# BaekMS/Sep-TFAnet-VAD

Hardware: AMD Instinct MI355X
Metric: utterances/sec/GPU (4s@8kHz, 2spk+VAD); SI-SDR within 0.01 dB of ref (higher is better)
Workload: dtype f16x3 (fp32-accurate); 1 GPU; cfg2 config_with_vad.json forward, B=64/GPU, N=32000 samples (4 s @ 8 kHz resampled to 16 kHz), T=126 frames; full forward: STFT, 24 TCN blocks, VAD, iSTFT, est (side attributes on read); global_batch=64, seq_len=32000, parallelism=dp1 (independent utterance shards, no data-path collective)

## Files before the change

sep-tfanet-vad_amd/csrc/api.hip:

```cpp
#include <hip/hip_runtime.h>
#include <hip/hip_fp16.h>

#include "build/build_id.h"

#include <algorithm>
#include <climits>
#include <cmath>
#include <cstdio>
#include <cstdlib>
#include <cstring>
#include <memory>
#include <mutex>
#include <numeric>
#include <string>
#include <unordered_map>
#include <vector>

#include <rocprofiler-sdk-roctx/roctx.h>

#include "../../include/sepvad.h"
#include "sepvad_internal.h"
#include "stoi_design.h"

using namespace sepvad;
// ... 48 lines not shown

Workspace ws_view(const Workspace& w, int b0, int Tp) {
  Workspace v = w;
  const size_t u = (size_t)b0 * Tp;
  v.X = w.X + u * NBIN; v.specdb = w.specdb + u * SPEC_LD; v.S0 = w.S0 + u * CH;
  v.O[0] = w.O[0] + u * CH; v.O[1] = w.O[1] + u * CH; v.A = w.A + u * CH; v.R = w.R + u * CH;
  v.masks = w.masks + u * MOUT_PAD;
  v.Dhi = w.Dhi + u * HID; v.Dlo = w.Dlo + u * HID; v.D32 = w.D32 + u * HID;
  v.colsum = w.colsum + u * (CH / TILE); v.rowsum = w.rowsum + (size_t)b0 * (Tp / TILE) * CH;
  v.at = w.at + u; v.af = w.af + (size_t)b0 * CH; v.vy = w.vy + u * 2 * 4; v.vad = w.vad + u * 2;
  v.vP = w.vP + u * 2 * HEAD_VAD_N;
  v.rec_gate = w.rec_gate + (size_t)b0 * (Tp / GATE_ROWS) * 2;
  v.rec_g1 = w.rec_g1 + (size_t)b0 * (Tp / TILE) * (CH / TILE) * 2;
  v.rec_dw = w.rec_dw + (size_t)b0 * (Tp / STAT_ROWS) * 2;
  v.rec_mom = w.rec_mom + (size_t)b0 * (Tp / STAT_ROWS) * NMOM;
  v.rec_hs = w.rec_hs + (size_t)b0 * (Tp / STAT_ROWS) * 2;
  v.rec_vad = w.rec_vad + (size_t)b0 * 2 * (Tp / VAD_ROWS) * 2;
  return v;
}

constexpr int MAX_SPLIT = 4;
constexpr int TCLK_RECS = 4096;

struct StreamCtx {
  void* stream = nullptr;
  Workspace ws;
  unsigned long long* tgran = nullptr;
  unsigned* terr = nullptr;
  unsigned* herr = nullptr;
  unsigned* herr_dev = nullptr;
  unsigned reported = 0;
  unsigned pending = 0;
  unsigned tsalt = 0;
  int last_B = 0, last_N = 0;
  long long seq = 0;
  unsigned long long used = 0;
};

}

struct sepvad_model {
  SepVadConfig cfg{};
  int device = 0;
  int nblk = 0;
  int prec = PREC_F16X3;
  float* dparams = nullptr;
  __half* dhalf = nullptr;
  std::vector<BlockOff> blk;
  size_t win_in = 0, win_out = 0, win_inv = 0, tw = 0;
  size_t ln_g = 0, ln_b = 0;
  PackedW wout;
  size_t out_g = 0, out_b = 0, bo = 0;
  PackedW wout_spk, vadw;
  size_t bo_spk = 0, out_nyw = 0, out_nyb = 0, vad_ny = 0;
  float vad_sx = 1.f;
  float out_a = 0.f;
  size_t v_w1 = 0, v_b1 = 0, v_g = 0, v_b = 0, v_w2 = 0;
  float v_a = 0.f, v_b2 = 0.f;
  size_t gate = 0;
  bool same_stft_window = true;
  int split = 1;
  hipStream_t sub[MAX_SPLIT] = {};
  hipEvent_t fork = nullptr, join[MAX_SPLIT] = {};
  bool fused = true;
  int tcn_cap = 0;
  int tcn_cap_p[4] = {};
  __half* twf = nullptr;
  __half* twq[3] = {};
  __half* twfq = nullptr;
  int lo8 = 2;
  int tcn_cap_q[3] = {};
  int tcn2_cap_p[4] = {};
  int tcn2_cap_q[3] = {};
  int gran_slots = 0;
  __half* twf16 = nullptr;
  __half* twbf = nullptr;
  float* twf32 = nullptr;
  float* tprm = nullptr;
  bool last_fused = false;
  float out_sx = 1.f;
  int last_nsl = 1;
  float* tdump = nullptr;
  std::vector<std::unique_ptr<StreamCtx>> ctx;
  std::mutex mu;
  unsigned long long use_clock = 0;
  long long fwd_seq = 0;
  int res_B = 0, res_N = 0;
  unsigned long long* kprobe = nullptr;
  unsigned long long* tprobe = nullptr;
  unsigned long long* tclk = nullptr;
  long long tclk_n = 0;
  bool timing = false;
  std::vector<hipEvent_t> ev;
  double gemm_ms = 0.0, g2_ms = 0.0, total_ms = 0.0;
  int gemm_launches = 0, g2_launches = 0;
  int probe_blk = -1;
  unsigned long long* probe = nullptr;
  size_t probe_n = 0;

  const float* P(size_t off) const { return dparams + off; }
  const __half* H(size_t off) const { return dhalf + off; }
};

namespace {

struct TensorMap {
  std::unordered_map<std::string, std::pair<const float*, int64_t>> m;
// ... 614 lines not shown
        const float* bb = get(q + convs[j] + ".bias", 1);
        BAIL();
        attp[4 * j + 0] = w[0]; attp[4 * j + 1] = w[1]; attp[4 * j + 2] = w[2]; attp[4 * j + 3] = bb[0];
      }
      const float* pt = get(q + ".prelu_t.weight", 1);
      const float* pf = get(q + ".prelu_f.weight", 1);
      BAIL();
      attp[16] = pt[0]; attp[17] = pf[0];
    }
    bo.attp = pk.add(attp);
    if (c.ln_mode == SEPVAD_LN_RECURSIVE) {
      const float* fa = get("TCN.ln_first_modules." + std::to_string(i) + ".weight", CH);
      const float* fb = get("TCN.ln_first_modules." + std::to_string(i) + ".bias", CH);
      const float* sa = get("TCN.ln_second_modules." + std::to_string(i) + ".weight", CH);
      const float* sb = get("TCN.ln_second_modules." + std::to_string(i) + ".bias", CH);
      BAIL();
      bo.lna_g = pk.add(fa, CH); bo.lna_b = pk.add(fb, CH);
      bo.lnb_g = pk.add(sa, CH); bo.lnb_b = pk.add(sb, CH);
      xbound = gn_bound(sa, sb, CH);
      for (int j = 0; j < 5; ++j) bo.wsum[j] = 0.0;
      for (int k = 0; k < CH; ++k) {
        const double g = fa[k], e = fb[k];
        bo.wsum[0] += g; bo.wsum[1] += e; bo.wsum[2] += e * e; bo.wsum[3] += g * e; bo.wsum[4] += g * g;
      }
    } else if (c.ln_mode == SEPVAD_LN_RESIDUAL) {
      const float* fa = get("TCN.ln_modules." + std::to_string(i) + ".weight", CH);
      const float* fb = get("TCN.ln_modules." + std::to_string(i) + ".bias", CH);
      BAIL();
      bo.lna_g = pk.add(fa, CH); bo.lna_b = pk.add(fb, CH);
      xbound += gn_bound(fa, fb, CH);
    } else {
      xbound = 0.0;
    }
    h->blk.push_back(bo);
  }
  {
    const float* oa = get("TCN.output.0.weight", 1);
    const float* og = get("TCN.output.1.weight", CH);
    const float* ob = get("TCN.output.1.bias", CH);
    const float* gg = get("TCN.output.2.weight_g", MOUT);
    const float* vv = get("TCN.output.2.weight_v", (int64_t)MOUT * CH);
    const float* bb = get("TCN.output.2.bias", MOUT);
    BAIL();
    h->out_a = oa[0];
    h->out_g = pk.add(og, CH);
    h->out_b = pk.add(ob, CH);
    const int eh = range_exp(gn_bound(og, ob, CH));
    h->out_sx = std::ldexp(1.f, -eh);
    const std::vector<float> wo = fold_wn(gg, vv, MOUT, CH);
    h->wout = pack_pointwise(pk, wo, MOUT, CH, MOUT_PAD, eh);
    std::vector<float> bpad(MOUT_PAD, 0.f);
    std::memcpy(bpad.data(), bb, MOUT * sizeof(float));
    h->bo = pk.add(bpad);
    std::vector<float> ws((size_t)MOUT_PAD * CH, 0.f), bs(MOUT_PAD, 0.f);
    for (int q = 0; q < 2; ++q)
      for (int i = 0; i < NBIN; ++i) {
        std::memcpy(&ws[((size_t)q * HEAD_SPK + i) * CH], &wo[((size_t)q * NBIN + i) * CH], CH * sizeof(float));
        bs[q * HEAD_SPK + i] = bb[q * NBIN + i];
      }
    h->wout_spk = pack_pointwise(pk, ws, MOUT_PAD, CH, MOUT_PAD, eh);
    h->bo_spk = pk.add(bs);
    std::vector<float> nyw((size_t)2 * CH), nyb(2);
    for (int q = 0; q < 2; ++q) {
      std::memcpy(&nyw[(size_t)q * CH], &wo[((size_t)q * NBIN + NBIN - 1) * CH], CH * sizeof(float));
      nyb[q] = bb[q * NBIN + NBIN - 1];
    }
    h->out_nyw = pk.add(nyw);
    h->out_nyb = pk.add(nyb);
  }
  if (c.final_vad) {
    const float* g1 = get("vad.common.conv1_1.weight_g", 4);
    const float* v1 = get("vad.common.conv1_1.weight_v", (int64_t)4 * NBIN * 5);
    const float* b1 = get("vad.common.conv1_1.bias", 4);
    const float* a = get("vad.common.relu_1.weight", 1);
    const float* gg = get("vad.common.BN_1.weight", 4);
    const float* gb = get("vad.common.BN_1.bias", 4);
    const float* g2 = get("vad.output_layer_vad.weight_g", 1);
    const float* v2 = get("vad.output_layer_vad.weight_v", 12);
    const float* b2 = get("vad.output_layer_vad.bias", 1);
    BAIL();
    const std::vector<float> w1 = fold_wn(g1, v1, 4, NBIN * 5);
    h->v_w1 = pk.add(w1);
    std::vector<float> wv((size_t)32 * HEAD_SPK, 0.f);
    for (int o = 0; o < 4; ++o)
      for (int c2 = 0; c2 < NBIN; ++c2)
        for (int k = 0; k < 5; ++k) wv[(size_t)(4 * k + o) * HEAD_SPK + c2] = w1[((size_t)o * NBIN + c2) * 5 + k];
    double mb = 0.0;
    {
      const std::vector<float> wo = fold_wn(get("TCN.output.2.weight_g", MOUT), get("TCN.output.2.weight_v", (int64_t)MOUT * CH), MOUT, CH);
      const float* ob2 = get("TCN.output.2.bias", MOUT);
      const double ab = gn_bound(get("TCN.output.1.weight", CH), get("TCN.output.1.bias", CH), CH);
      for (int r = 0; r < MOUT; ++r) {
        double sr = 0.0;
        for (int i = 0; i < CH; ++i) sr += std::fabs((double)wo[(size_t)r * CH + i]);
        mb = std::max(mb, sr * ab + std::fabs((double)ob2[r]));
      }
    }
    const int ev_ = range_exp(mb);
    h->vad_sx = std::ldexp(1.f, -ev_);
    h->vadw = pack_pointwise(pk, wv, HEAD_VAD_N, HEAD_SPK, 32, ev_);
    std::vector<float> vny(HEAD_VAD_N);
    for (int o = 0; o < 4; ++o)
      for (int k = 0; k < 5; ++k) vny[4 * k + o] = w1[((size_t)o * NBIN + NBIN - 1) * 5 + k];
    h->vad_ny = pk.add(vny);
    h->v_b1 = pk.add(b1, 4);
    h->v_a = a[0];
    h->v_g = pk.add(gg, 4);
    h->v_b = pk.add(gb, 4);
    h->v_w2 = pk.add(fold_wn(g2, v2, 1, 12));
    h->v_b2 = b2[0];
  }
  {
    std::vector<float> gw(12, 0.f);
    if (c.activity_input) {
      const float* w = get("activity_input.weight", 9);
      const float* bb = get("activity_input.bias", 1);
      const float* pa = get("prelu.weight", 1);
      BAIL();
      std::memcpy(gw.data(), w, 9 * sizeof(float));
      gw[9] = bb[0];
      gw[10] = pa[0];
// ... 201 lines not shown
    sa.window_db = h->same_stft_window ? sa.window : h->P(h->win_in);
    sa.X = w.X;
    sa.specdb = h->same_stft_window ? nullptr : w.specdb;
    sa.activity = c.activity_input; sa.gate_w = h->P(h->gate);
    sa.S0 = w.S0; sa.gate_rec = w.rec_gate;
    TailProbe tp(h, s, kn, "stft");
    sa.probe = tp.buf;
    HIPCHK(launch_stft_gate(sa, s));
    HIPCHK(tp.dump(B, Tp / (2 * GATE_ROWS)));
    if (out->spectrum) {
      GateArgs ga{};
      ga.B = B; ga.T = T; ga.Tp = Tp; ga.activity = c.activity_input;
      ga.X = h->same_stft_window ? w.X : nullptr; ga.specdb = w.specdb; ga.w = h->P(h->gate);
      ga.S0 = nullptr; ga.out_rec = nullptr;
      ga.spec_side = out->spectrum + (size_t)b0 * NBIN * T;
      HIPCHK(launch_gate(ga, s));
    }
  }
  stage.next("sepvad::tcn_head");
  const int G = (T + FR - 1) / FR;
  const bool use_fused = fused_ok(h, T);
  unsigned gsalt_lo = 0, gsalt_n = 0;
  h->last_fused = use_fused;
  const bool has_vad = c.final_vad && (!c.final_vad_masked_speakers || c.noisy_phase);
  const bool vad_in_head = use_fused && has_vad && !c.final_vad_masked_speakers;
  if (use_fused) {
    const int nsl = h->tdump ? 1 : tcn_slices(h, kn, B, G);
    const int cap = nsl == 2 ? tcn2_cap_of(h) : tcn_cap_of(h);
    h->last_nsl = nsl;
    const int Gt = G / nsl;
    TcnArgs ta{};
    ta.T = T; ta.Tp = Tp; ta.G = G; ta.nsl = nsl; ta.nblk = h->nblk; ta.layer = c.layer;
    if (const int nb = kn.tcn_nblk; nb > 0 && nb < h->nblk) ta.nblk = nb;
    ta.ln_mode = ld_mode_of(c);
    ta.tf_att = c.tf_attention;
    ta.prec = h->prec;
    ta.lo8 = h->prec == PREC_F16X3 ? h->lo8 : 0;
    ta.wfrag = h->prec == PREC_F16X3 ? (ta.lo8 ? h->twq[ta.lo8] : h->twf)
                                     : (h->prec == PREC_F16 ? h->twf16
                                                            : (h->prec == PREC_F32 ? reinterpret_cast<const __half*>(h->twf32) : h->twbf));
    ta.prm = h->tprm;
    ta.inv_ch = 1.0 / ((double)CH * T);
    ta.inv_hid = 1.0 / ((double)HID * T);
    ta.alpha_h = h->out_a;
    ta.gran = cx->tgran; ta.err = cx->terr; ta.herr = cx->herr_dev;
    ta.xmode = kn.tcn_xmode;
    auto launch_t = [&](const TcnArgs& t, int grid) { return launch_tcn(t, grid, s); };
    ta.spin_limit = (unsigned)kn.tcn_spin_limit;
    ta.force_err = kn.tcn_force_giveup;
    ta.dbg_delay = (unsigned)std::max(0, kn.tcn_delay);
    ta.dump_blk = std::max(0, std::min(h->nblk - 1, kn.tcn_dump_block));
    int ngroups = std::min(B, cap / Gt);
    if (ngroups >= 8 && kn.tcn_align8) ngroups -= ngroups % 8;
    ta.hg = h->P(h->out_g); ta.hbe = h->P(h->out_b); ta.hsx = h->out_sx;
    ta.hwh = h->prec == PREC_F32 ? reinterpret_cast<const __half*>(h->P(h->wout_spk.ff32))
                                 : h->H(h->prec == PREC_BF16 ? h->wout_spk.fbf : h->wout_spk.fhi);
    ta.hwl = h->H(ta.lo8 == 2 ? h->wout_spk.fi8 : (ta.lo8 == 1 ? h->wout_spk.fl8 : h->wout_spk.flo));
    if (ta.lo8 == 2 && nsl == 2 && kn.tcn_wq16 >= 1 && h->tcn2_cap_p[PREC_F16X3] >= cap) {
      ta.lo8 = 0;
      ta.wfrag = h->twfq;
      ta.hwl = h->H(h->wout_spk.fq);
    }
    ta.hwscale = h->P(h->wout_spk.scale); ta.hbias = h->P(h->bo_spk);
    ta.hnyw = h->P(h->out_nyw); ta.hnyb = h->P(h->out_nyb);
    if (vad_in_head) {
      ta.hvwh = h->H(h->vadw.fhi); ta.hvwl = h->H(h->vadw.flo); ta.hvwscale = h->P(h->vadw.scale);
      ta.hvwf = h->P(h->vadw.ff32);
      ta.hvny = h->P(h->vad_ny);
      ta.hvsx = h->vad_sx;
    }
    if (const int mg = kn.tcn_max_groups; mg > 0 && mg < ngroups) ngroups = mg;
    ta.run = 0;
    if (nsl == 1 && G > 32) {
      const int R = (G + 7) / 8;
      if (std::min(B, cap / (8 * R)) >= ngroups) ta.run = R;
    }
    const int gstride = ta.run ? 8 * ta.run : Gt;
    const int ep_utt = 4 * h->nblk + 1;
    int max_iter = ((1 << TCN_EPOCH_BITS) - 2) / ep_utt;
    if (const int mi = kn.tcn_max_iter) max_iter = std::min(max_iter, mi);
    if (max_iter < 1) return fail(SEPVAD_E_ARG, "fused TCN: too many blocks");
    if (1 + (long long)max_iter * ep_utt >= (1 << TCN_EPOCH_BITS)) return fail(SEPVAD_E_ARG, "fused TCN: epoch budget");
    const int per_launch = max_iter * ngroups;
    const char* probe_path = kn.tcn_probe;
    const size_t probe_n = (size_t)h->tcn_cap * h->nblk * 16 * 9;
    const bool warm = probe_path && kn.tcn_probe_warm;
    {
      const int rc = salt_reserve(h, cx, s, kn, (unsigned)((B + per_launch - 1) / per_launch + (warm ? 1 : 0)), &gsalt_lo);
      if (rc) return rc;
    }
    gsalt_n = 0;
    for (int u0 = 0; u0 < B; u0 += per_launch) {
      const int Bl = std::min(per_launch, B - u0);
      const int ng = std::min(ngroups, Bl);
      const int ngl = ng;
      ta.tag0 = (gsalt_lo + gsalt_n++) << TCN_EPOCH_BITS;
      ta.B = Bl;
      ta.S0 = w.S0 + (size_t)u0 * Tp * CH;
      ta.ln = gn_src(w.rec_gate + (size_t)u0 * (Tp / GATE_ROWS) * 2, Tp / GATE_ROWS, 2, 0, h->P(h->ln_g), h->P(h->ln_b), 1e-8f);
      ta.hmasks = w.masks + (size_t)u0 * Tp * MOUT_PAD;
      ta.hvP = vad_in_head ? w.vP + (size_t)u0 * 2 * Tp * HEAD_VAD_N : nullptr;
      ta.probe = nullptr;
      ta.dump = (h->tdump && u0 == 0 && Bl == B) ? h->tdump : nullptr;
      if (probe_path && u0 == 0) {
        if (!h->tprobe) HIPCHK(hipMalloc(&h->tprobe, probe_n * sizeof(unsigned long long)));
        HIPCHK(hipMemsetAsync(h->tprobe, 0, probe_n * sizeof(unsigned long long), s));
        ta.probe = h->tprobe;
        if (warm) {
          TcnArgs tw = ta;
          tw.probe = nullptr;
          HIPCHK(launch_t(tw, ngl * gstride));
          ta.tag0 = (gsalt_lo + gsalt_n++) << TCN_EPOCH_BITS;
        }
      }
      ta.clk = nullptr;
      if (kn.tcn_clock) {
        if (!h->tclk) {
// ... 761 lines not shown
```

sep-tfanet-vad_amd/csrc/sepvad_internal.h:

```cpp
#pragma once
#include <hip/hip_runtime.h>
#include <hip/hip_fp16.h>
#include <cstdint>

namespace sepvad {

constexpr int NFFT = 512;
constexpr int HOP = 256;
constexpr int NBIN = 257;
constexpr int CH = 256;
constexpr int HID = 512;
constexpr int TILE = 64;
constexpr int MOUT = 2 * NBIN;
constexpr int MOUT_PAD = 576;
constexpr int HEAD_SPK = MOUT_PAD / 2;
constexpr int HEAD_VAD_N = 20;
constexpr int SPEC_LD = 260;
constexpr int STAT_ROWS = 8;
constexpr int PROBE_SLOTS = 16;
constexpr int NMOM = 11;

inline int round_up(int a, int b) { return (a + b - 1) / b * b; }

enum Precision { PREC_F32 = 0, PREC_F16X3 = 1, PREC_F16 = 2, PREC_BF16 = 3 };
// ... 274 lines not shown
constexpr int FR = 32;
#ifndef SEPVAD_FG_MAX
#define SEPVAD_FG_MAX 256
#endif
constexpr int FG_MAX = SEPVAD_FG_MAX;
constexpr int FG_CHUNK = 8;
constexpr int FG_WAVE = 16;
constexpr int NGR = 2624;
#ifndef SEPVAD_FG_TREE
#define SEPVAD_FG_TREE 16
#endif
constexpr int FG_TREE = SEPVAD_FG_TREE;
constexpr int TCN_EPOCH_BITS = 12;
constexpr int PB_WS1 = 0, PB_B1 = 256, PB_G1 = 512, PB_BE1 = 768;
constexpr int PB_WD = 1024, PB_BD = 2560;
constexpr int PB_WS2 = 3072, PB_B2 = 3328, PB_FC2 = 3584;
constexpr int PB_LNAG = 3840, PB_LNAB = 4096, PB_LNBG = 4352, PB_LNBB = 4608;
constexpr int PB_ATT = 4864;
constexpr int PB_A1 = 4884, PB_A2 = 4885;
constexpr int PB_SX = 4886, PB_SXN = 4887;
constexpr int PB_WSUM = 4888;
constexpr int PB_EPS2 = 4898;
constexpr int PB_SFC2 = 4899, PB_SB2 = 4900;
constexpr int PB_SIZE = 4904;
constexpr size_t WF_W1L = 65536, WF_W2H = 131072, WF_W2L = 262144, WF_BLOCK = 393216;
constexpr size_t WS_W2 = 65536, WS_BLOCK = 196608;
constexpr size_t WS32_W2 = 2 * 65536, WS32_BLOCK = 2 * 196608;
constexpr size_t WQ_W1L = 65536, WQ_W2H = 98304, WQ_W2L = 229376, WQ_BLOCK = 294912;
constexpr int WQ_LO_SHIFT = 19;
struct TcnArgs {
  int B, T, Tp, G, nblk, layer, ln_mode, tf_att, prec;
  int nsl;
  int run;
  int lo8;
  const __half* wfrag;
  const float* prm;
  const float* S0;
  GnSrc ln;
  float alpha_h;
  unsigned long long* gran;
  unsigned tag0;
  unsigned* err;
  unsigned* herr;
  unsigned spin_limit;
  int force_err;
  double inv_ch, inv_hid;
  int xmode;
  unsigned long long* probe;
  unsigned long long* clk;
  float* dump;
  unsigned dbg_delay;
  int dump_blk;
  float* hmasks;
  const float* hg; const float* hbe;
  float hsx;
  const __half* hwh; const __half* hwl;
  const float* hwscale; const float* hbias;
  const float* hnyw; const float* hnyb;
  const __half* hvwh; const __half* hvwl; const float* hvwscale; const float* hvny;
  const float* hvwf;
  float hvsx;
  float* hvP;
  unsigned long long* hprobe;
};
hipError_t launch_tcn(const TcnArgs& a, int grid, hipStream_t s);
int tcn_blocks_per_cu(int ln_mode, int prec, int lo, int nsl = 1);
uint8_t e4m3_rn(float x);

hipError_t launch_gemm(const GemmArgs& a, int ep, hipStream_t s);
hipError_t launch_dw_stats(const DwStatsArgs& a, hipStream_t s);
hipError_t launch_att_stats(const AttStatsArgs& a, hipStream_t s);
hipError_t launch_head_stats(const HeadStatsArgs& a, hipStream_t s);
hipError_t launch_gate(const GateArgs& a, hipStream_t s);
struct MaskSideArgs {
  int B, T, Tp;
  const float* masks;
  float* masks_b;
  float* mask;
};
hipError_t launch_mask_side(const MaskSideArgs& a, hipStream_t s);
hipError_t launch_stft(const StftArgs& a, hipStream_t s);
hipError_t launch_vad1(const Vad1Args& a, hipStream_t s);
hipError_t launch_istft(const IstftArgs& a, hipStream_t s);
hipError_t launch_istft_pair(const IstftArgs& a, hipStream_t s);

}
```

sep-tfanet-vad_amd/csrc/tcn_kernel.h:

```cpp
#pragma once
#include <type_traits>

#include "tcn_common.h"

namespace sepvad {

#ifndef TCN_SUB
#define TCN_SUB 0
#endif

constexpr int NTHR = 512;
constexpr int LDX = CH + 8;
constexpr int LDD = HID + 8;
constexpr int HROW = FR + 8;
constexpr int LDXF = CH + 4;
constexpr int LDDF = HID + 4;
#ifndef TCN_PD
#define TCN_PD 8
#endif
constexpr int PD = TCN_PD;
#ifndef TCN_DIAG
#define TCN_DIAG 0
#endif
#ifndef TCN_PDQ
// ... 1000 lines not shown
          if (tid < nw) sm.gw[tid] = v[0];
        } else {
          const int nw = 2 * NMOM * G;
          if (!LG || nw <= NTHR) {
            const u64* pp[1] = {tid < nw ? slot(tid / (2 * NMOM), e4) + GW_P4 + tid % (2 * NMOM) : nullptr};
            unsigned v[1];
            gpoll<1>(pp, tag4, v, a);
            if (tid < nw) sm.gw[tid] = v[0];
          } else for (int k0 = 0; k0 < nw; k0 += 4 * NTHR) {
            const u64* pp[4];
            unsigned v[4];
#pragma unroll
            for (int j = 0; j < 4; ++j) {
              const int k = k0 + tid + j * NTHR;
              pp[j] = k < nw ? slot(k / (2 * NMOM), e4) + GW_P4 + k % (2 * NMOM) : nullptr;
            }
            gpoll<4>(pp, tag4, v, a);
#pragma unroll
            for (int j = 0; j < 4; ++j) {
              const int k = k0 + tid + j * NTHR;
              if (k < nw) sm.gw[k] = v[j];
            }
          }
        }
      TPROBE(11);
        __syncthreads();
        const double* gd = reinterpret_cast<const double*>(sm.gw);
        const double sj = seq_sum_lds(gd + (lane < NMOM ? lane : 0), NMOM, tree ? nlead : G);
        double ms[NMOM];
#pragma unroll
        for (int j = 0; j < NMOM; ++j) ms[j] = readlane_d(sj, j);
        if constexpr (LM == LD_RECURSIVE) {
          float mua, rsa, mub, rsb;
          recursive_moments_f(ms, reinterpret_cast<const double*>(pm + PB_WSUM), 1e-5f, 1e-5f, a.inv_ch, (double)T, mua,
                              rsa, mub, rsb);
          kc[0] = rsa * pm[PB_LNAG + m]; kc[1] = pm[PB_LNAB + m] - kc[0] * mua;
          kc[2] = rsb * pm[PB_LNBG + m]; kc[3] = pm[PB_LNBB + m] - kc[2] * mub;
        } else {
          float mu, rs;
          gn_moments_f(ms[2], ms[3], a.inv_ch, 1e-5f, mu, rs);
          kc[0] = rs * pm[PB_LNAG + m]; kc[1] = pm[PB_LNAB + m] - kc[0] * mu;
        }
      if (TCN_SUB == 0) TPROBE(13);
      }
      const bool lastb = bi + 1 == a.nblk;
      const int hjl = (wave_s + (blockIdx.x >> 3)) & 7;
      const __amdgpu_buffer_rsrc_t wnh = lastb ? rsrc_of(a.hwh) : rsrc_of(wb + WL::BLOCK);
      const __amdgpu_buffer_rsrc_t wnl = lastb ? rsrc_of(PRE == PREC_F16X3 ? a.hwl : a.hwh) : rsrc_of(wb + WL::BLOCK + WL::W1L);
      const int pvo = lastb ? (hjl * NS1 * 64 + lane) * VB : voff1;
      const int pvol = lastb ? (F32 ? pvo + 16 : (hjl * (NS1 / 2) * 64 + lane) * 16) : voff1l;
      if (TCN_SUB == 0) TPROBE(14);
      {
        const float sxn = pm[PB_SXN];
        auto xup_rows = [&](auto MPC) {
        constexpr int MP = decltype(MPC)::value;
#pragma unroll
        for (int r = 0; r < 16 * NSL; r += 2) {
          const int pr = r / 2;
          if (NSL == 1 || pr % 2 == 0) {
#pragma unroll
            for (int e = 0; e < RPI; ++e) prefetch_w1<PRE, RD, LQ>(wnh, wnl, pvo, pvol, rh, rl, RPI * (pr / NSL) + e);
          }
          const int tl = trow(r);
          const f32x2 x = resid_apply2<LM>(f32x2{o[r], o[r + 1]}, f32x2{rv[r >> 4][r & 15], rv[r >> 4][(r & 15) + 1]},
                                           kc);
          const f32x2 vm = r / 2 < 8 * NSL - MP ? f32x2{1.f, 1.f}
                                                : f32x2{t0 + tl < T ? 1.f : 0.f, t0 + tl + 1 < T ? 1.f : 0.f};
          const f32x2 ov = x * vm;
          o[r] = ov.x; o[r + 1] = ov.y;
          split_store_rows_pk<PRE>(sm.Ahi, sm.Alo, tl * LDXE + m, LDXE, ov * sxn, (lane & 1) != 0);
        }
        };
        by_mp(xup_rows);
      }
      __syncthreads();
      TPROBE(12);
    }
    {
      const int tidh = fresh_tid(wave_s);
      const int hl4h = 4 * ((tidh >> 5) & 1), mh = 32 * wave_s + (tidh & 31);
      auto trow = [&](int r) { return FR * (r >> 4) + (r & 3) + 8 * ((r & 15) >> 2) + hl4h; };
      unsigned long long* const hpr = a.hprobe != nullptr && u == grp ? a.hprobe + (size_t)blockIdx.x * 8 : nullptr;
      auto hstamp = [&](int k) {
        if (hpr != nullptr && tidh == 0) hpr[k] = __builtin_amdgcn_s_memtime();
      };
      if (hpr != nullptr && tidh == 0) hpr[0] = wall_clock64();
      hstamp(1);
      const int jl = (wave_s + (blockIdx.x >> 3)) & 7;
      const __amdgpu_buffer_rsrc_t wh = rsrc_of(a.hwh), wl = rsrc_of(PRE == PREC_F16X3 ? a.hwl : a.hwh);
      {
        float st[2 * NSL];
#pragma unroll
        for (int k = 0; k < 2 * NSL; ++k) st[k] = 0.f;
#pragma unroll
        for (int r = 0; r < 16 * NSL; ++r) {
          if (t0 + trow(r) < T) {
            const float pv = prelu_f(o[r], a.alpha_h);
            st[2 * (r >> 4)] += pv; st[2 * (r >> 4) + 1] += pv * pv;
          }
        }
        block_sums<2 * NSL>(st, sm.red, sm.dred, tidh);
      }
      const unsigned e5 = ++ep, tag5 = a.tag0 + e5;
      if (tidh < 2 * NSL)
        gputd(slot(m0 + (tidh >> 1), e5) + GW_STAT + 2 * (tidh & 1), tag5, sm.dred[tidh], l2);
      {
        constexpr int NP = LG ? 2 : 1;
        const u64* p[NP];
        unsigned v[NP];
        p[0] = tidh < 4 * G ? slot(tidh >> 2, e5) + GW_STAT + (tidh & 3) : nullptr;
        if constexpr (LG) p[NP - 1] = tidh + NTHR < 4 * G ? slot((tidh + NTHR) >> 2, e5) + GW_STAT + (tidh & 3) : nullptr;
        gpoll<NP>(p, tag5, v, a);
        if (tidh < 4 * G) sm.gw[tidh] = v[0];
        if constexpr (LG) if (tidh + NTHR < 4 * G) sm.gw[tidh + NTHR] = v[NP - 1];
      }
      hstamp(2);
      __syncthreads();
      if (tidh < 2) {
        const double* gd = reinterpret_cast<const double*>(sm.gw);
        sm.dred[8 + tidh] = seq_sum_lds(gd + tidh, 2, G);
      }
      __syncthreads();
      {
        float mu, rs;
        gn_moments_f(sm.dred[8], sm.dred[9], a.inv_ch, 1e-5f, mu, rs);
        const float sc = rs * a.hg[mh], sh = a.hbe[mh] - sc * mu;
#pragma unroll
        for (int r = 0; r < 16 * NSL; ++r)
          split_store<PRE>(sm.Ahi, sm.Alo, trow(r) * LDXE + mh, fmaf(prelu_f(o[r], a.alpha_h), sc, sh) * a.hsx);
      }
      __syncthreads();
      hstamp(3);
      const bool vad = a.hvP != nullptr;
      float* const vsc = F32 ? reinterpret_cast<float*>(sm.Alo) + wave_s * FR * 32
                             : (NSL == 1 ? reinterpret_cast<float*>((wave_s < 4 ? sm.Ahi : sm.Alo) + FR * LDX) + (wave_s & 3) * FR * 32
                                         : sm.H + 16 * FR * HEAD_VAD_N + wave_s * FR * 32);
      float* const Ps = sm.H;
      auto vidx = [](int t, int c) { return t * 32 + ((((c >> 2) ^ t) & 7) << 2) + (c & 3); };
      float* const nys = NSL == 1 ? &sm.c[0][0] : reinterpret_cast<float*>(sm.gw);
#pragma unroll 1
      for (int sl = 0; sl < NSL; ++sl) {
        const int tidh = fresh_tid(wave_s), lh = tidh & 63, hl4h = 4 * ((tidh >> 5) & 1);
        auto trow1 = [&](int r) { return (r & 3) + 8 * (r >> 2) + hl4h; };
        auto tile_voff = [&](int q) { return ((q * (HEAD_SPK / 32) + jl) * NS1 * 64 + lh) * VB; };
        auto tile_voffl = [&](int q) { return F32 ? tile_voff(q) + 16 : ((q * (HEAD_SPK / 32) + jl) * (NS1 / 2) * 64 + lh) * 16; };
#pragma unroll
        for (int q = 0; q < 2; ++q) {
          const int jt = q * (HEAD_SPK / 32) + jl;
          f32x16v acc[1];
#pragma unroll
          for (int r = 0; r < 16; ++r) acc[0][r] = 0.f;
          wave_gemm<NS1, LDXE, PRE, RD, LQ>(acc, plane_at<PRE>(sm.Ahi, FR * sl * LDXE), plane_at<PRE>(sm.Alo, FR * sl * LDXE),
                                            wh, wl, tile_voff(q), tile_voffl(q), rh, rl, lh);
          if (q == 0) prefetch_w<PRE, RD, LQ>(wh, wl, tile_voff(1), tile_voffl(1), rh, rl);
          else if (sl + 1 < NSL) prefetch_w<PRE, RD, LQ>(wh, wl, tile_voff(0), tile_voffl(0), rh, rl);
          f16x8 vb[2][2];
          if (vad && !F32) {
#pragma unroll
            for (int st = 0; st < 2; ++st) {
              vb[st][0] = *reinterpret_cast<const f16x8*>(a.hvwh + ((size_t)(2 * jl + st) * 64 + lh) * 8);
              vb[st][1] = *reinterpret_cast<const f16x8*>(a.hvwl + ((size_t)(2 * jl + st) * 64 + lh) * 8);
            }
          }
          const int c = 32 * jl + (lh & 31);
          const float ws = a.hwscale[32 * jt + (lh & 31)], bias = a.hbias[32 * jt + (lh & 31)];
          float* const out = a.hmasks + ((size_t)u * Tp + t0 + FR * sl) * MOUT_PAD + q * NBIN + c;
#pragma unroll
          for (int r = 0; r < 16; ++r) {
            acc[0][r] = fmaf(acc[0][r], ws, bias);
            st_out(out + (size_t)trow1(r) * MOUT_PAD, acc[0][r]);
          }
          if (vad) {
#pragma unroll
            for (int r = 0; r < 16; ++r) vsc[vidx(trow1(r), lh & 31)] = acc[0][r] * a.hvsx;
            wave_lds_sync();
            f32x16v pv;
#pragma unroll
            for (int r = 0; r < 16; ++r) pv[r] = 0.f;
#pragma unroll
            for (int st = 0; st < 2; ++st) {
              const int tr = lh & 31, c0 = 16 * st + 8 * (lh >> 5);
              const f32x4 x0 = *reinterpret_cast<const f32x4*>(vsc + vidx(tr, c0));
              const f32x4 x1 = *reinterpret_cast<const f32x4*>(vsc + vidx(tr, c0 + 4));
              if constexpr (F32) {
                const float* wf = a.hvwf + ((size_t)(2 * jl + st) * 64 + lh) * 8;
                const f32x4 b0 = *reinterpret_cast<const f32x4*>(wf), b1 = *reinterpret_cast<const f32x4*>(wf + 4);
#pragma unroll
                for (int j = 0; j < 4; ++j) pv = __builtin_amdgcn_mfma_f32_32x32x2f32(x0[j], b0[j], pv, 0, 0, 0);
#pragma unroll
                for (int j = 0; j < 4; ++j) pv = __builtin_amdgcn_mfma_f32_32x32x2f32(x1[j], b1[j], pv, 0, 0, 0);
                continue;
              }
              f16x8 ah, al;
#pragma unroll
              for (int e = 0; e < 8; ++e) {
                const float x = e < 4 ? x0[e] : x1[e - 4];
                const _Float16 hh = (_Float16)x;
                ah[e] = hh;
                al[e] = (_Float16)(x - (float)hh);
              }
              pv = __builtin_amdgcn_mfma_f32_32x32x16_f16(al, vb[st][0], pv, 0, 0, 0);
              pv = __builtin_amdgcn_mfma_f32_32x32x16_f16(ah, vb[st][1], pv, 0, 0, 0);
              pv = __builtin_amdgcn_mfma_f32_32x32x16_f16(ah, vb[st][0], pv, 0, 0, 0);
            }
            wave_lds_sync();
            if ((lh & 31) < HEAD_VAD_N) {
#pragma unroll
              for (int r = 0; r < 16; ++r) Ps[((jl * 2 + q) * FR + trow1(r)) * HEAD_VAD_N + (lh & 31)] = pv[r];
            }
          }
        }
        if (sl + 1 == NSL) hstamp(4);
        {
          const int od = tidh >> 3, part = tidh & 7, qn = od >> 5, tn = od & 31;
          const _Float16* ah = sm.Ahi + (FR * sl + tn) * LDX + 32 * part;
          const _Float16* al = sm.Alo + (FR * sl + tn) * LDX + 32 * part;
          const f32x4* wq = reinterpret_cast<const f32x4*>(a.hnyw + qn * CH + 32 * part);
          float sn = 0.f;
#pragma unroll
          for (int k = 0; k < 4; ++k) {
            float xv[8];
            if constexpr (F32) {
              const float* af = reinterpret_cast<const float*>(sm.Ahi) + (FR * sl + tn) * LDXE + 32 * part + 8 * k;
              const f32x4 u0 = *reinterpret_cast<const f32x4*>(af), u1 = *reinterpret_cast<const f32x4*>(af + 4);
#pragma unroll
              for (int e = 0; e < 8; ++e) xv[e] = e < 4 ? u0[e] : u1[e - 4];
            } else if constexpr (PRE == PREC_BF16) {
              const bf16x8 bv = *reinterpret_cast<const bf16x8*>(reinterpret_cast<const __bf16*>(ah) + 8 * k);
#pragma unroll
              for (int e = 0; e < 8; ++e) xv[e] = (float)bv[e];
            } else {
              const f16x8 hv = *reinterpret_cast<const f16x8*>(ah + 8 * k);
              f16x8 lv = {};
              if constexpr (PRE == PREC_F16X3) lv = *reinterpret_cast<const f16x8*>(al + 8 * k);
#pragma unroll
              for (int e = 0; e < 8; ++e) xv[e] = PRE == PREC_F16X3 ? (float)hv[e] + (float)lv[e] : (float)hv[e];
            }
            const f32x4 w0 = wq[2 * k], w1 = wq[2 * k + 1];
#pragma unroll
            for (int e = 0; e < 8; ++e) sn = fmaf(xv[e], e < 4 ? w0[e] : w1[e - 4], sn);
          }
          sn += __shfl_xor(sn, 1);
          sn += __shfl_xor(sn, 2);
          sn += __shfl_xor(sn, 4);
          if (part == 0) nys[qn * FR + tn] = sn / a.hsx + a.hnyb[qn];
        }
        __syncthreads();
        const int ts = t0 + FR * sl;
        for (int i = tidh; i < (vad ? 2 * FR * HEAD_VAD_N : 2 * FR); i += NTHR) {
          const int per = vad ? FR * HEAD_VAD_N : FR;
          const int q = i >= per ? 1 : 0, ri = i - q * per;
          const int t = vad ? ri / HEAD_VAD_N : ri, n = vad ? ri - t * HEAD_VAD_N : 0;
          const float m = nys[q * FR + t];
          if (n == 0) st_out(a.hmasks + ((size_t)u * Tp + ts + t) * MOUT_PAD + q * NBIN + (NBIN - 1), m);
          if (vad) {
            float sum = 0.f;
#pragma unroll
            for (int w = 0; w < 8; ++w) sum += Ps[((w * 2 + q) * FR + t) * HEAD_VAD_N + n];
            a.hvP[(((size_t)u * 2 + q) * Tp + ts) * HEAD_VAD_N + ri] = ts + t < T ? fmaf(m, a.hvny[n], sum * a.hvwscale[n]) : 0.f;
          }
        }
        if (sl + 1 == NSL) hstamp(5);
        __syncthreads();
      }
    }
  }
  if (unsigned long long* const ck = kargs()->clk; ck != nullptr && threadIdx.x == 0) {
    const unsigned long long rt = wall_clock64();
    if (blockIdx.x == 0) { ck[3] = rt; ck[5] = __builtin_amdgcn_s_memtime(); }
    __hip_atomic_fetch_max(ck + 1, rt, __ATOMIC_RELAXED, __HIP_MEMORY_SCOPE_AGENT);
  }
}

template <int PRE, int LQ, bool LG>
static hipError_t launch_tcn_pre(const TcnArgs& a, int grid, hipStream_t s) {
  if constexpr (PRE == PREC_F16X3) {
    if (a.dump != nullptr) {
      switch (a.ln_mode) {
        case LD_RECURSIVE: hipLaunchKernelGGL((k_tcn<LD_RECURSIVE, PRE, true, LQ, false, LG>), dim3(grid), dim3(NTHR), 0, s, a); break;
        case LD_RESIDUAL: hipLaunchKernelGGL((k_tcn<LD_RESIDUAL, PRE, true, LQ, false, LG>), dim3(grid), dim3(NTHR), 0, s, a); break;
        case LD_ADD: hipLaunchKernelGGL((k_tcn<LD_ADD, PRE, true, LQ, false, LG>), dim3(grid), dim3(NTHR), 0, s, a); break;
        default: return hipErrorInvalidValue;
      }
      return hipGetLastError();
    }
  }
  if (a.probe != nullptr && a.ln_mode == LD_RECURSIVE) {
    hipLaunchKernelGGL((k_tcn<LD_RECURSIVE, PRE, false, LQ, true, LG>), dim3(grid), dim3(NTHR), 0, s, a);
    return hipGetLastError();
  }
  switch (a.ln_mode) {
    case LD_RECURSIVE: hipLaunchKernelGGL((k_tcn<LD_RECURSIVE, PRE, false, LQ, false, LG>), dim3(grid), dim3(NTHR), 0, s, a); break;
    case LD_RESIDUAL: hipLaunchKernelGGL((k_tcn<LD_RESIDUAL, PRE, false, LQ, false, LG>), dim3(grid), dim3(NTHR), 0, s, a); break;
    case LD_ADD: hipLaunchKernelGGL((k_tcn<LD_ADD, PRE, false, LQ, false, LG>), dim3(grid), dim3(NTHR), 0, s, a); break;
    default: return hipErrorInvalidValue;
  }
  return hipGetLastError();
}

template <int PRE, int LQ>
static hipError_t launch_tcn2_pre(const TcnArgs& a, int grid, hipStream_t s) {
  if (a.dump != nullptr) return hipErrorInvalidValue;
  if (a.probe != nullptr && a.ln_mode == LD_RECURSIVE) {
    hipLaunchKernelGGL((k_tcn<LD_RECURSIVE, PRE, false, LQ, true, false, 2>), dim3(grid), dim3(NTHR), 0, s, a);
    return hipGetLastError();
  }
  switch (a.ln_mode) {
    case LD_RECURSIVE: hipLaunchKernelGGL((k_tcn<LD_RECURSIVE, PRE, false, LQ, false, false, 2>), dim3(grid), dim3(NTHR), 0, s, a); break;
    case LD_RESIDUAL: hipLaunchKernelGGL((k_tcn<LD_RESIDUAL, PRE, false, LQ, false, false, 2>), dim3(grid), dim3(NTHR), 0, s, a); break;
    case LD_ADD: hipLaunchKernelGGL((k_tcn<LD_ADD, PRE, false, LQ, false, false, 2>), dim3(grid), dim3(NTHR), 0, s, a); break;
    default: return hipErrorInvalidValue;
  }
// ... 33 lines not shown
```

Before: 142,600 utterances/s.

## Fold output GroupNorm affine into head weights and overlap moment wait with GEMM

The output GroupNorm's gamma and beta are folded algebraically into the head projection: the per-row constants c1 = W·gamma and c2 = W·beta + bias are precomputed on the host. This lets the head GEMM run on the unnormalized PReLU activations, which are written to LDS during the last block's update pass together with their partial moments. The mean and rstd are then applied after the GEMM as a per-row scale and offset. This removes a separate normalize-and-restore pass over the activations and moves the global-moment poll behind the first GEMM tile, so the cross-block wait overlaps with compute. It also hoists weight, scale and VAD loads ahead of the loop and switches output writes to raw buffer stores. The risks are precision loss from applying the normalization after an fp16 split GEMM with a new range scale, and added register pressure.

```diff
diff --git a/sep-tfanet-vad_amd/csrc/api.hip b/sep-tfanet-vad_amd/csrc/api.hip
--- a/sep-tfanet-vad_amd/csrc/api.hip
+++ b/sep-tfanet-vad_amd/csrc/api.hip
@@ -124,7 +124,8 @@
   PackedW wout;
   size_t out_g = 0, out_b = 0, bo = 0;
   PackedW wout_spk, vadw;
-  size_t bo_spk = 0, out_nyw = 0, out_nyb = 0, vad_ny = 0;
+  size_t c1_spk = 0, c2_spk = 0, out_nyw = 0, out_nyc = 0, vad_ny = 0;
+  float outp_sx = 1.f;
   float vad_sx = 1.f;
   float out_a = 0.f;
   size_t v_w1 = 0, v_b1 = 0, v_g = 0, v_b = 0, v_w2 = 0;
@@ -845,21 +846,34 @@
     std::vector<float> bpad(MOUT_PAD, 0.f);
     std::memcpy(bpad.data(), bb, MOUT * sizeof(float));
     h->bo = pk.add(bpad);
-    std::vector<float> ws((size_t)MOUT_PAD * CH, 0.f), bs(MOUT_PAD, 0.f);
-    for (int q = 0; q < 2; ++q)
-      for (int i = 0; i < NBIN; ++i) {
-        std::memcpy(&ws[((size_t)q * HEAD_SPK + i) * CH], &wo[((size_t)q * NBIN + i) * CH], CH * sizeof(float));
-        bs[q * HEAD_SPK + i] = bb[q * NBIN + i];
+    double gmax = 0.0;
+    for (int k = 0; k < CH; ++k) gmax = std::max(gmax, std::fabs((double)og[k]));
+    const int ehp = range_exp(gmax * xbound * std::max(1.0, std::fabs((double)oa[0])));
+    h->outp_sx = std::ldexp(1.f, -ehp);
+    std::vector<float> ws((size_t)MOUT_PAD * CH, 0.f), c1s(MOUT_PAD, 0.f), c2s(MOUT_PAD, 0.f);
+    std::vector<float> nyw((size_t)2 * CH), nyc(4);
+    auto fold_row = [&](const float* w, float bias, float* wg, float& c1, float& c2) {
+      double s1 = 0.0, s2 = bias;
+      for (int k = 0; k < CH; ++k) {
+        wg[k] = w[k];
+        s1 += (double)w[k] * og[k];
+        s2 += (double)w[k] * ob[k];
       }
-    h->wout_spk = pack_pointwise(pk, ws, MOUT_PAD, CH, MOUT_PAD, eh);
-    h->bo_spk = pk.add(bs);
-    std::vector<float> nyw((size_t)2 * CH), nyb(2);
+      c1 = (float)s1;
+      c2 = (float)s2;
+    };
     for (int q = 0; q < 2; ++q) {
-      std::memcpy(&nyw[(size_t)q * CH], &wo[((size_t)q * NBIN + NBIN - 1) * CH], CH * sizeof(float));
-      nyb[q] = bb[q * NBIN + NBIN - 1];
-    }
+      for (int i = 0; i < NBIN; ++i)
+        fold_row(&wo[((size_t)q * NBIN + i) * CH], bb[q * NBIN + i], &ws[((size_t)q * HEAD_SPK + i) * CH],
+                 c1s[q * HEAD_SPK + i], c2s[q * HEAD_SPK + i]);
+      fold_row(&wo[((size_t)q * NBIN + NBIN - 1) * CH], bb[q * NBIN + NBIN - 1], &nyw[(size_t)q * CH], nyc[2 * q],
+               nyc[2 * q + 1]);
+    }
+    h->wout_spk = pack_pointwise(pk, ws, MOUT_PAD, CH, MOUT_PAD, ehp);
+    h->c1_spk = pk.add(c1s);
+    h->c2_spk = pk.add(c2s);
     h->out_nyw = pk.add(nyw);
-    h->out_nyb = pk.add(nyb);
+    h->out_nyc = pk.add(nyc);
   }
   if (c.final_vad) {
     const float* g1 = get("vad.common.conv1_1.weight_g", 4);
@@ -1167,7 +1181,7 @@
     ta.dump_blk = std::max(0, std::min(h->nblk - 1, kn.tcn_dump_block));
     int ngroups = std::min(B, cap / Gt);
     if (ngroups >= 8 && kn.tcn_align8) ngroups -= ngroups % 8;
-    ta.hg = h->P(h->out_g); ta.hbe = h->P(h->out_b); ta.hsx = h->out_sx;
+    ta.hg = h->P(h->out_g); ta.hsx = h->outp_sx;
     ta.hwh = h->prec == PREC_F32 ? reinterpret_cast<const __half*>(h->P(h->wout_spk.ff32))
                                  : h->H(h->prec == PREC_BF16 ? h->wout_spk.fbf : h->wout_spk.fhi);
     ta.hwl = h->H(ta.lo8 == 2 ? h->wout_spk.fi8 : (ta.lo8 == 1 ? h->wout_spk.fl8 : h->wout_spk.flo));
@@ -1176,8 +1190,8 @@
       ta.wfrag = h->twfq;
       ta.hwl = h->H(h->wout_spk.fq);
     }
-    ta.hwscale = h->P(h->wout_spk.scale); ta.hbias = h->P(h->bo_spk);
-    ta.hnyw = h->P(h->out_nyw); ta.hnyb = h->P(h->out_nyb);
+    ta.hwscale = h->P(h->wout_spk.scale); ta.hc1 = h->P(h->c1_spk); ta.hc2 = h->P(h->c2_spk);
+    ta.hnyw = h->P(h->out_nyw); ta.hnyc = h->P(h->out_nyc);
     if (vad_in_head) {
       ta.hvwh = h->H(h->vadw.fhi); ta.hvwl = h->H(h->vadw.flo); ta.hvwscale = h->P(h->vadw.scale);
       ta.hvwf = h->P(h->vadw.ff32);
diff --git a/sep-tfanet-vad_amd/csrc/sepvad_internal.h b/sep-tfanet-vad_amd/csrc/sepvad_internal.h
--- a/sep-tfanet-vad_amd/csrc/sepvad_internal.h
+++ b/sep-tfanet-vad_amd/csrc/sepvad_internal.h
@@ -350,11 +350,11 @@
   unsigned dbg_delay;
   int dump_blk;
   float* hmasks;
-  const float* hg; const float* hbe;
+  const float* hg;
   float hsx;
   const __half* hwh; const __half* hwl;
-  const float* hwscale; const float* hbias;
-  const float* hnyw; const float* hnyb;
+  const float* hwscale; const float* hc1; const float* hc2;
+  const float* hnyw; const float* hnyc;
   const __half* hvwh; const __half* hvwl; const float* hvwscale; const float* hvny;
   const float* hvwf;
   float hvsx;
diff --git a/sep-tfanet-vad_amd/csrc/tcn_kernel.h b/sep-tfanet-vad_amd/csrc/tcn_kernel.h
--- a/sep-tfanet-vad_amd/csrc/tcn_kernel.h
+++ b/sep-tfanet-vad_amd/csrc/tcn_kernel.h
@@ -1076,8 +1076,10 @@
       if (TCN_SUB == 0) TPROBE(14);
       {
         const float sxn = pm[PB_SXN];
-        auto xup_rows = [&](auto MPC) {
+        auto xup_rows = [&](auto MPC, auto LBC, float (&s5)[2 * NSL]) {
         constexpr int MP = decltype(MPC)::value;
+        constexpr bool LB = decltype(LBC)::value;
+        const float ah = LB ? kargs()->alpha_h : 0.f, hsx = LB ? kargs()->hg[m] * kargs()->hsx : 0.f;
 #pragma unroll
         for (int r = 0; r < 16 * NSL; r += 2) {
           const int pr = r / 2;
@@ -1092,19 +1094,39 @@
                                                 : f32x2{t0 + tl < T ? 1.f : 0.f, t0 + tl + 1 < T ? 1.f : 0.f};
           const f32x2 ov = x * vm;
           o[r] = ov.x; o[r + 1] = ov.y;
-          split_store_rows_pk<PRE>(sm.Ahi, sm.Alo, tl * LDXE + m, LDXE, ov * sxn, (lane & 1) != 0);
+          if constexpr (LB) {
+            const f32x2 p = {prelu_f(ov.x, ah), prelu_f(ov.y, ah)};
+            float& s = s5[2 * (r >> 4)];
+            float& ss = s5[2 * (r >> 4) + 1];
+            s += p.x; ss = fmaf(p.x, p.x, ss);
+            s += p.y; ss = fmaf(p.y, p.y, ss);
+            split_store_rows_pk<PRE>(sm.Ahi, sm.Alo, tl * LDXE + m, LDXE, p * hsx, (lane & 1) != 0);
+          } else {
+            split_store_rows_pk<PRE>(sm.Ahi, sm.Alo, tl * LDXE + m, LDXE, ov * sxn, (lane & 1) != 0);
+          }
         }
         };
-        by_mp(xup_rows);
-      }
-      __syncthreads();
+        if (!lastb) {
+          float none[2 * NSL];
+          by_mp([&](auto MPC) { xup_rows(MPC, std::false_type{}, none); });
+          __syncthreads();
+        } else {
+          float s5[2 * NSL];
+#pragma unroll
+          for (int k = 0; k < 2 * NSL; ++k) s5[k] = 0.f;
+          by_mp([&](auto MPC) { xup_rows(MPC, std::true_type{}, s5); });
+          block_sums<2 * NSL>(s5, sm.red, sm.dred, tid);
+          const unsigned e5 = ++ep;
+          if (tid < 2 * NSL)
+            gputd(slot(m0 + (tid >> 1), e5) + GW_STAT + 2 * (tid & 1), a.tag0 + e5, sm.dred[tid], l2);
+        }
+      }
       TPROBE(12);
     }
     {
       const int tidh = fresh_tid(wave_s);
-      const int hl4h = 4 * ((tidh >> 5) & 1), mh = 32 * wave_s + (tidh & 31);
-      auto trow = [&](int r) { return FR * (r >> 4) + (r & 3) + 8 * ((r & 15) >> 2) + hl4h; };
-      unsigned long long* const hpr = a.hprobe != nullptr && u == grp ? a.hprobe + (size_t)blockIdx.x * 8 : nullptr;
+      const KArgs ka = kargs();
+      unsigned long long* const hpr = ka->hprobe != nullptr && u == grp ? ka->hprobe + (size_t)blockIdx.x * 8 : nullptr;
       auto hstamp = [&](int k) {
         if (hpr != nullptr && tidh == 0) hpr[k] = __builtin_amdgcn_s_memtime();
       };
@@ -1112,91 +1134,111 @@
       hstamp(1);
       const int jl = (wave_s + (blockIdx.x >> 3)) & 7;
       const __amdgpu_buffer_rsrc_t wh = rsrc_of(a.hwh), wl = rsrc_of(PRE == PREC_F16X3 ? a.hwl : a.hwh);
-      {
-        float st[2 * NSL];
-#pragma unroll
-        for (int k = 0; k < 2 * NSL; ++k) st[k] = 0.f;
-#pragma unroll
-        for (int r = 0; r < 16 * NSL; ++r) {
-          if (t0 + trow(r) < T) {
-            const float pv = prelu_f(o[r], a.alpha_h);
-            st[2 * (r >> 4)] += pv; st[2 * (r >> 4) + 1] += pv * pv;
-          }
-        }
-        block_sums<2 * NSL>(st, sm.red, sm.dred, tidh);
-      }
-      const unsigned e5 = ++ep, tag5 = a.tag0 + e5;
-      if (tidh < 2 * NSL)
-        gputd(slot(m0 + (tidh >> 1), e5) + GW_STAT + 2 * (tidh & 1), tag5, sm.dred[tidh], l2);
-      {
+      auto p5_moments = [&]() {
+        const unsigned e5 = ep, tag5 = a.tag0 + e5;
         constexpr int NP = LG ? 2 : 1;
         const u64* p[NP];
         unsigned v[NP];
         p[0] = tidh < 4 * G ? slot(tidh >> 2, e5) + GW_STAT + (tidh & 3) : nullptr;
         if constexpr (LG) p[NP - 1] = tidh + NTHR < 4 * G ? slot((tidh + NTHR) >> 2, e5) + GW_STAT + (tidh & 3) : nullptr;
         gpoll<NP>(p, tag5, v, a);
-        if (tidh < 4 * G) sm.gw[tidh] = v[0];
-        if constexpr (LG) if (tidh + NTHR < 4 * G) sm.gw[tidh + NTHR] = v[NP - 1];
-      }
-      hstamp(2);
-      __syncthreads();
-      if (tidh < 2) {
-        const double* gd = reinterpret_cast<const double*>(sm.gw);
-        sm.dred[8 + tidh] = seq_sum_lds(gd + tidh, 2, G);
-      }
-      __syncthreads();
-      {
-        float mu, rs;
-        gn_moments_f(sm.dred[8], sm.dred[9], a.inv_ch, 1e-5f, mu, rs);
-        const float sc = rs * a.hg[mh], sh = a.hbe[mh] - sc * mu;
-#pragma unroll
-        for (int r = 0; r < 16 * NSL; ++r)
-          split_store<PRE>(sm.Ahi, sm.Alo, trow(r) * LDXE + mh, fmaf(prelu_f(o[r], a.alpha_h), sc, sh) * a.hsx);
-      }
-      __syncthreads();
-      hstamp(3);
-      const bool vad = a.hvP != nullptr;
+        if constexpr (!LG) {
+          if (wave_s == 0) {
+            float mu, rs;
+            member_moments_w(v[0], 0, G, a.inv_ch, 1e-5f, mu, rs);
+            if ((tidh & 63) == 0) { sm.gmom[0] = mu; sm.gmom[1] = rs; }
+          }
+        } else {
+          if (tidh < 4 * G) sm.gw[tidh] = v[0];
+          if (tidh + NTHR < 4 * G) sm.gw[tidh + NTHR] = v[NP - 1];
+          __syncthreads();
+          if (tidh < 2) {
+            const double* gd = reinterpret_cast<const double*>(sm.gw);
+            sm.dred[8 + tidh] = seq_sum_lds(gd + tidh, 2, G);
+          }
+          __syncthreads();
+          if (tidh == 0) {
+            float mu, rs;
+            gn_moments_f(sm.dred[8], sm.dred[9], a.inv_ch, 1e-5f, mu, rs);
+            sm.gmom[0] = mu; sm.gmom[1] = rs;
+          }
+        }
+      };
+      const bool vad = ka->hvP != nullptr;
       float* const vsc = F32 ? reinterpret_cast<float*>(sm.Alo) + wave_s * FR * 32
                              : (NSL == 1 ? reinterpret_cast<float*>((wave_s < 4 ? sm.Ahi : sm.Alo) + FR * LDX) + (wave_s & 3) * FR * 32
                                          : sm.H + 16 * FR * HEAD_VAD_N + wave_s * FR * 32);
       float* const Ps = sm.H;
       auto vidx = [](int t, int c) { return t * 32 + ((((c >> 2) ^ t) & 7) << 2) + (c & 3); };
       float* const nys = NSL == 1 ? &sm.c[0][0] : reinterpret_cast<float*>(sm.gw);
+      float* const hvs = sm.red + 32;
+      static_assert(32 + 2 * 32 <= sizeof(sm.red) / sizeof(float) && HEAD_VAD_N <= 32 && 2 * NSL * 8 <= 32, "staged tap-sum values");
+      float hvq = 0.f;
+      if (vad && tidh < 2 * HEAD_VAD_N) hvq = (tidh < HEAD_VAD_N ? ka->hvny : ka->hvwscale - HEAD_VAD_N)[tidh];
+      float hrs = 0.f, hrm = 0.f;
 #pragma unroll 1
       for (int sl = 0; sl < NSL; ++sl) {
         const int tidh = fresh_tid(wave_s), lh = tidh & 63, hl4h = 4 * ((tidh >> 5) & 1);
         auto trow1 = [&](int r) { return (r & 3) + 8 * (r >> 2) + hl4h; };
         auto tile_voff = [&](int q) { return ((q * (HEAD_SPK / 32) + jl) * NS1 * 64 + lh) * VB; };
         auto tile_voffl = [&](int q) { return F32 ? tile_voff(q) + 16 : ((q * (HEAD_SPK / 32) + jl) * (NS1 / 2) * 64 + lh) * 16; };
+        float tws[2], tc1[2], tc2[2];
+        f16x8 vb[2][2];
+        __builtin_amdgcn_sched_barrier(0);
 #pragma unroll
         for (int q = 0; q < 2; ++q) {
-          const int jt = q * (HEAD_SPK / 32) + jl;
+          const int row = 32 * (q * (HEAD_SPK / 32) + jl) + (lh & 31);
+          tws[q] = ka->hwscale[row]; tc1[q] = ka->hc1[row]; tc2[q] = ka->hc2[row];
+        }
+        if (vad && !F32) {
+#pragma unroll
+          for (int st = 0; st < 2; ++st) {
+            vb[st][0] = *reinterpret_cast<const f16x8*>(ka->hvwh + ((size_t)(2 * jl + st) * 64 + lh) * 8);
+            vb[st][1] = *reinterpret_cast<const f16x8*>(ka->hvwl + ((size_t)(2 * jl + st) * 64 + lh) * 8);
+          }
+        }
+        __builtin_amdgcn_sched_barrier(0);
+        const int od = tidh >> 3, part = tidh & 7, qn = od >> 5, tn = od & 31;
+        float nyc1 = 0.f, nyc2 = 0.f;
+#pragma unroll
+        for (int q = 0; q < 2; ++q) {
           f32x16v acc[1];
 #pragma unroll
           for (int r = 0; r < 16; ++r) acc[0][r] = 0.f;
           wave_gemm<NS1, LDXE, PRE, RD, LQ>(acc, plane_at<PRE>(sm.Ahi, FR * sl * LDXE), plane_at<PRE>(sm.Alo, FR * sl * LDXE),
                                             wh, wl, tile_voff(q), tile_voffl(q), rh, rl, lh);
-          if (q == 0) prefetch_w<PRE, RD, LQ>(wh, wl, tile_voff(1), tile_voffl(1), rh, rl);
-          else if (sl + 1 < NSL) prefetch_w<PRE, RD, LQ>(wh, wl, tile_voff(0), tile_voffl(0), rh, rl);
-          f16x8 vb[2][2];
-          if (vad && !F32) {
-#pragma unroll
-            for (int st = 0; st < 2; ++st) {
-              vb[st][0] = *reinterpret_cast<const f16x8*>(a.hvwh + ((size_t)(2 * jl + st) * 64 + lh) * 8);
-              vb[st][1] = *reinterpret_cast<const f16x8*>(a.hvwl + ((size_t)(2 * jl + st) * 64 + lh) * 8);
-            }
+          if (q == 0) {
+            prefetch_w<PRE, RD, LQ>(wh, wl, tile_voff(1), tile_voffl(1), rh, rl);
+            __builtin_amdgcn_sched_barrier(0);
+            nyc1 = ka->hnyc[2 * qn]; nyc2 = ka->hnyc[2 * qn + 1];
+            __builtin_amdgcn_sched_barrier(0);
+            if (sl == 0) {
+              hstamp(2);
+              p5_moments();
+              if (vad && tidh < 2 * HEAD_VAD_N) hvs[tidh < HEAD_VAD_N ? tidh : 32 + tidh - HEAD_VAD_N] = hvq;
+              __syncthreads();
+              const float mu = sm.gmom[0];
+              hrs = sm.gmom[1];
+              hrm = hrs * mu;
+              hstamp(3);
+            }
+          } else if (sl + 1 < NSL) {
+            prefetch_w<PRE, RD, LQ>(wh, wl, tile_voff(0), tile_voffl(0), rh, rl);
           }
           const int c = 32 * jl + (lh & 31);
-          const float ws = a.hwscale[32 * jt + (lh & 31)], bias = a.hbias[32 * jt + (lh & 31)];
-          float* const out = a.hmasks + ((size_t)u * Tp + t0 + FR * sl) * MOUT_PAD + q * NBIN + c;
-#pragma unroll
-          for (int r = 0; r < 16; ++r) {
-            acc[0][r] = fmaf(acc[0][r], ws, bias);
-            st_out(out + (size_t)trow1(r) * MOUT_PAD, acc[0][r]);
-          }
+          const float ws = tws[q] * hrs, kq = fmaf(-hrm, tc1[q], tc2[q]);
+          const __amdgpu_buffer_rsrc_t outr = rsrc_of(ka->hmasks + ((size_t)u * Tp + t0 + FR * sl) * MOUT_PAD);
+          const int outv = (hl4h * MOUT_PAD + q * NBIN + c) * 4;
+          float mv[16];
+#pragma unroll
+          for (int r = 0; r < 16; ++r) mv[r] = fmaf(acc[0][r], ws, kq);
+#pragma unroll
+          for (int r = 0; r < 16; ++r)
+            __builtin_amdgcn_raw_buffer_store_b32(__builtin_bit_cast(unsigned, mv[r]), outr, outv,
+                                                  ((r & 3) + 8 * (r >> 2)) * MOUT_PAD * 4, 0);
           if (vad) {
 #pragma unroll
-            for (int r = 0; r < 16; ++r) vsc[vidx(trow1(r), lh & 31)] = acc[0][r] * a.hvsx;
+            for (int r = 0; r < 16; ++r) vsc[vidx(trow1(r), lh & 31)] = mv[r] * ka->hvsx;
             wave_lds_sync();
             f32x16v pv;
 #pragma unroll
@@ -1207,7 +1249,7 @@
               const f32x4 x0 = *reinterpret_cast<const f32x4*>(vsc + vidx(tr, c0));
               const f32x4 x1 = *reinterpret_cast<const f32x4*>(vsc + vidx(tr, c0 + 4));
               if constexpr (F32) {
-                const float* wf = a.hvwf + ((size_t)(2 * jl + st) * 64 + lh) * 8;
+                const float* wf = ka->hvwf + ((size_t)(2 * jl + st) * 64 + lh) * 8;
                 const f32x4 b0 = *reinterpret_cast<const f32x4*>(wf), b1 = *reinterpret_cast<const f32x4*>(wf + 4);
 #pragma unroll
                 for (int j = 0; j < 4; ++j) pv = __builtin_amdgcn_mfma_f32_32x32x2f32(x0[j], b0[j], pv, 0, 0, 0);
@@ -1236,10 +1278,9 @@
         }
         if (sl + 1 == NSL) hstamp(4);
         {
-          const int od = tidh >> 3, part = tidh & 7, qn = od >> 5, tn = od & 31;
           const _Float16* ah = sm.Ahi + (FR * sl + tn) * LDX + 32 * part;
           const _Float16* al = sm.Alo + (FR * sl + tn) * LDX + 32 * part;
-          const f32x4* wq = reinterpret_cast<const f32x4*>(a.hnyw + qn * CH + 32 * part);
+          const f32x4* wq = reinterpret_cast<const f32x4*>(ka->hnyw + qn * CH + 32 * part);
           float sn = 0.f;
 #pragma unroll
           for (int k = 0; k < 4; ++k) {
@@ -1267,7 +1308,7 @@
           sn += __shfl_xor(sn, 1);
           sn += __shfl_xor(sn, 2);
           sn += __shfl_xor(sn, 4);
-          if (part == 0) nys[qn * FR + tn] = sn / a.hsx + a.hnyb[qn];
+          if (part == 0) nys[qn * FR + tn] = fmaf(sn / ka->hsx, hrs, fmaf(-hrm, nyc1, nyc2));
         }
         __syncthreads();
         const int ts = t0 + FR * sl;
@@ -1276,12 +1317,12 @@
           const int q = i >= per ? 1 : 0, ri = i - q * per;
           const int t = vad ? ri / HEAD_VAD_N : ri, n = vad ? ri - t * HEAD_VAD_N : 0;
           const float m = nys[q * FR + t];
-          if (n == 0) st_out(a.hmasks + ((size_t)u * Tp + ts + t) * MOUT_PAD + q * NBIN + (NBIN - 1), m);
+          if (n == 0) st_out(ka->hmasks + ((size_t)u * Tp + ts + t) * MOUT_PAD + q * NBIN + (NBIN - 1), m);
           if (vad) {
             float sum = 0.f;
 #pragma unroll
             for (int w = 0; w < 8; ++w) sum += Ps[((w * 2 + q) * FR + t) * HEAD_VAD_N + n];
-            a.hvP[(((size_t)u * 2 + q) * Tp + ts) * HEAD_VAD_N + ri] = ts + t < T ? fmaf(m, a.hvny[n], sum * a.hvwscale[n]) : 0.f;
+            ka->hvP[(((size_t)u * 2 + q) * Tp + ts) * HEAD_VAD_N + ri] = ts + t < T ? fmaf(m, hvs[n], sum * hvs[32 + n]) : 0.f;
           }
         }
         if (sl + 1 == NSL) hstamp(5);
```

Result: slower. 139,500 utterances/s (-2.2%).
